# audexdev/Lossless-Audio-Codec

Measured on AMD Instinct MI355X. Metric: encode Msamples/s at 1/2/4/8 MI355X; byte-identical .lac vs CPU ref, higher is better.
Workload: dtype int64

## Files before the change

### include/lacx.h

```cpp
#ifndef LACX_H
#define LACX_H
#include <stddef.h>
#include <stdint.h>

#ifdef __cplusplus
extern "C" {
#endif

#define LACX_OK 0
#define LACX_E_INVALID 1
#define LACX_E_RUNTIME 2
#define LACX_E_DEVICE 3
#define LACX_E_MISMATCH 4

#define LACX_MAX_BLOCK 16384u
#define LACX_SLOTS_PER_BLOCK 16u

typedef struct lacx_encoder lacx_encoder;

typedef struct lacx_config {
    uint32_t sample_rate;
    uint8_t bit_depth;
    uint8_t stereo_mode;
    uint8_t zero_run_enabled;
// ... 31 lines not shown
    double h2d_ms;
    double analysis_ms;
    double ingest_ms;
    double probe_ms;
    double full_ms;
    double d2h_ms;
    double emit_ms;
    double total_ms;
    uint64_t full_slots;
    uint64_t probe_slots;
    uint32_t full_launches;
    uint32_t regrows;
    double full_exec_ms;
    uint32_t emit_direct;
    uint32_t moved_by_k_pack;
    uint32_t packer_gave_up;
    uint32_t drain_copies;
    double drain_first_ms;
    double drain_last_ms;
    double poll_gap_max_ms;
    double kernels_done_ms;
    double enqueue_ms;
    uint32_t silent_copies;
    uint32_t reserved0;
} lacx_timing;

int lacx_encoder_create(const lacx_config* cfg, lacx_encoder** out);
void lacx_encoder_destroy(lacx_encoder* enc);
const char* lacx_last_error(const lacx_encoder* enc);
void lacx_free(void* p);
void lacx_get_timing(const lacx_encoder* enc, lacx_timing* out);

uint32_t lacx_sizeof(const char* struct_name);

int lacx_encode(lacx_encoder* enc, const int32_t* left, const int32_t* right, uint64_t frames,
                uint8_t** out, uint64_t* out_size);

int lacx_encode_device(lacx_encoder* enc, const int32_t* d_left, const int32_t* d_right,
                       const int32_t* h_left, const int32_t* h_right, uint64_t frames, void* stream,
                       uint8_t** out, uint64_t* out_size);

int lacx_analyze(lacx_encoder* enc, const int32_t* left, const int32_t* right, uint64_t frames,
                 lacx_block_plan* bplans, lacx_channel_plan* plans);
int lacx_analyze_device(lacx_encoder* enc, const int32_t* d_left, const int32_t* d_right, uint64_t frames,
                        void* stream, lacx_block_plan* bplans, lacx_channel_plan* plans);

int lacx_emit_from_plans(lacx_encoder* enc, const int32_t* left, const int32_t* right, uint64_t frames,
// ... 305 lines not shown
```

### lossless-audio-codec_amd/csrc/api_core.cpp

```cpp
#include "encoder_impl.h"

namespace lacx_host {

Knobs read_knobs() {
    Knobs k;
    auto set = [](const char* name) {
        const char* v = std::getenv(name);
        return v != nullptr;
    };
    auto num = [](const char* name) -> unsigned long long {
        const char* v = std::getenv(name);
        return v ? std::strtoull(v, nullptr, 0) : 0ull;
    };
    k.stream_priority = !set("LACX_NO_STREAM_PRIORITY");
    if (const char* v = std::getenv("LACX_FUSED_EMIT")) k.fused_emit = *v != '0';
    k.direct_packer = set("LACX_DIRECT_PACKER");
    k.packer = !set("LACX_NO_PACKER");
    k.persistent = !set("LACX_NO_PERSISTENT");
    k.debug_drain = set("LACX_DEBUG_DRAIN");
    k.two_copy_streams = !set("LACX_ONE_COPY_STREAM");
    if (const char* v = std::getenv("LACX_STREAM_PRIO")) {
        int a = 0, b = 0, c = 0;
        if (std::sscanf(v, "%d,%d,%d", &a, &b, &c) == 3) {
            k.prio_main = a;
            k.prio_chunks = b;
            k.prio_pack = c;
        }
    }
    k.front_halves = !set("LACX_NO_FRONT_HALVES");
    k.tune.fold_front = !set("LACX_NO_FRONT_FOLD");
    k.lazy_repair = !set("LACX_NO_LAZY_REPAIR");
    k.silent_template = !set("LACX_NO_SILENT_TEMPLATE");
    k.pinned_cap_bytes = num("LACX_PINNED_CAP_BYTES");
    k.debug_skip = (uint32_t)num("LACX_DEBUG_SKIP");
    k.pipe_chunks = (uint32_t)num("LACX_PIPE_CHUNKS");
    if (const char* v = std::getenv("LACX_PIPE_SPLIT")) k.pipe_split = v;
    k.drain_fence = (uint32_t)num("LACX_DRAIN_FENCE");
    if (const char* v = std::getenv("LACX_FANOUT_EXCHANGE")) k.fanout_exchange = std::strcmp(v, "host") == 0 ? 1u : (std::strcmp(v, "rccl") == 0 ? 2u : 0u);
    k.tune.persistent_grid = (uint32_t)num("LACX_PERSISTENT_GRID");
    k.tune.pack_nap = (int)num("LACX_PACK_NAP");
    k.tune.pack_grid = (int)num("LACX_PACK_GRID");
    k.tune.no_pairs = set("LACX_NO_PAIRS");
    return k;
}

double ms_since(clk::time_point t0) { return std::chrono::duration<double, std::milli>(clk::now() - t0).count(); }

int fail(lacx_encoder* e, int code, const std::string& msg) {
    if (e) e->err = msg;
    return code;
}

int hip_fail(lacx_encoder* e, hipError_t err, const char* what) {
    return fail(e, LACX_E_DEVICE, std::string(what) + ": " + hipGetErrorString(err));
}

void big_copy(uint8_t* dst, const uint8_t* src, uint64_t n) {
    constexpr uint64_t kPiece = 4ull << 20;
    const unsigned hw = std::thread::hardware_concurrency();
    const uint64_t want = std::min<uint64_t>(std::min<uint64_t>(8, hw ? hw : 1), n / kPiece);
    if (want < 2) {
        std::memcpy(dst, src, n);
        return;
    }
    std::vector<std::thread> pool;
// ... 401 lines not shown
```

### lossless-audio-codec_amd/csrc/api_fanout.cpp

```cpp
#include <dlfcn.h>

#include <atomic>
#include <barrier>
#include <functional>
#include <mutex>

#include "encoder_impl.h"

namespace {
using ncclComm_t = struct ncclComm*;
using ncclResult_t = int;
constexpr int kNcclUint64 = 5;
struct Rccl {
    void* lib = nullptr;
    ncclResult_t (*CommInitAll)(ncclComm_t*, int, const int*) = nullptr;
    ncclResult_t (*CommDestroy)(ncclComm_t) = nullptr;
    ncclResult_t (*AllGather)(const void*, void*, size_t, int, ncclComm_t, hipStream_t) = nullptr;
    const char* (*GetErrorString)(ncclResult_t) = nullptr;
};
Rccl* rccl() {
    static std::mutex mu;
    static Rccl r;
    static bool tried = false;
    std::lock_guard<std::mutex> lock(mu);
// ... 202 lines not shown
    const uint32_t by_size = std::max<uint32_t>(1u, nb / std::max<uint32_t>(1u, f.min_blocks));
    return std::max<uint32_t>(1u, std::min<uint32_t>((uint32_t)f.lanes.size(), std::min(by_size, nb)));
}

void merge_timing(lacx_encoder* e, uint32_t G, clk::time_point t0) {
    lacx_timing t{};
    for (uint32_t g = 0; g < G; ++g) {
        const lacx_timing& c = e->fan->lanes[g]->enc->timing;
        t.h2d_ms = std::max(t.h2d_ms, c.h2d_ms);
        t.analysis_ms = std::max(t.analysis_ms, c.analysis_ms);
        t.ingest_ms = std::max(t.ingest_ms, c.ingest_ms);
        t.probe_ms = std::max(t.probe_ms, c.probe_ms);
        t.full_ms = std::max(t.full_ms, c.full_ms);
        t.d2h_ms = std::max(t.d2h_ms, c.d2h_ms);
        t.emit_ms = std::max(t.emit_ms, c.emit_ms);
        t.full_exec_ms = std::max(t.full_exec_ms, c.full_exec_ms);
        t.full_slots += c.full_slots;
        t.probe_slots += c.probe_slots;
        t.full_launches = std::max(t.full_launches, c.full_launches);
        t.regrows += c.regrows;
        t.emit_direct += c.emit_direct;
        t.moved_by_k_pack += c.moved_by_k_pack;
        t.silent_copies += c.silent_copies;
        t.packer_gave_up += c.packer_gave_up;
    }
    t.total_ms = ms_since(t0);
    e->timing = t;
}

}

namespace lacx_host {

bool is_fanout(const lacx_encoder* e) { return e && e->fan; }

void destroy_fanout(lacx_encoder* e) {
    if (!e->fan) return;
    Fanout* f = e->fan;
    for (size_t g = 0; g < f->lanes.size(); ++g) {
        Lane& ln = *f->lanes[g];
        ln.worker.reset();
        if (ln.comm) {
            if (Rccl* r = rccl()) (void)r->CommDestroy(ln.comm);
        }
        if (ln.d_x || ln.h_x) {
            (void)hipSetDevice(ln.device);
// ... 211 lines not shown
```

### lossless-audio-codec_amd/csrc/api_pipeline.cpp

```cpp
#include "encoder_impl.h"

namespace lacx_host {

int enqueue_chunk(lacx_encoder* e, const int32_t* d_left, const int32_t* d_right, uint64_t frames, int channels,
                  int stereo_mode, int bit_depth, const Chunk& ck, int c, hipStream_t st) {
    const uint64_t f0 = (uint64_t)ck.first * kMaxBlock;
    const uint64_t f1 = std::min<uint64_t>(frames, (uint64_t)(ck.first + ck.count) * kMaxBlock);
    const AnalyzeParams prm = make_params(e, f1 - f0, channels, stereo_mode, bit_depth);
    const DeviceWorkspace w = ws_at(e->ws, ck.first);
    LaunchSet ls = one_stream_set(prm, d_left + f0, d_right ? d_right + f0 : nullptr);
    HIP_TRY(e, launch_analysis(bind(ls), w, st, e->ev[c]), "kernel launch");
    HIP_TRY(e, hipMemcpyAsync(e->h_plans + (size_t)ck.first * kSlotsPerBlock, w.plans,
                              (size_t)ck.count * kSlotsPerBlock * sizeof(ChannelPlan), hipMemcpyDeviceToHost, st),
            "D2H plans");
    HIP_TRY(e, hipMemcpyAsync(e->h_bplans + ck.first, w.bplans, (size_t)ck.count * sizeof(BlockPlan),
                              hipMemcpyDeviceToHost, st),
            "D2H block plans");
    HIP_TRY(e, hipEventRecord(e->done[c], st), "event record");
    return LACX_OK;
}

int analyze_on_device(lacx_encoder* e, const int32_t* d_left, const int32_t* d_right, uint64_t frames,
                      int channels, int stereo_mode, int bit_depth, hipStream_t st) {
    const uint32_t nb = blocks_for(frames);
// ... 162 lines not shown
bool gather_list(lacx_encoder* e, const DeviceWorkspace& w, const GatherJob& j, GatherList& g) {
    bool ok = true;
    auto map_if = [&](bool wanted, auto* host) {
        auto* m = wanted ? mapped(host) : nullptr;
        ok = ok && (m || !wanted);
        return m;
    };
    BlockPlan* m_bplans = map_if(j.what & kGatherBplans, e->h_bplans);
    uint32_t* m_table = map_if(j.what & kGatherTable, e->h_table());
    unsigned long long* m_sizes = map_if(j.what & kGatherSizes, e->h_sizes());
    unsigned long long* m_totals = map_if(j.what & (kGatherTotal | kGatherSizes), e->h_totals);
    uint32_t* m_err = map_if(true, e->h_err);
    uint32_t* m_emitted = map_if(j.items != 0, e->h_emitted());
    unsigned long long* m_tspan = map_if(j.what & kGatherTspan, e->h_tspan);
    if (!ok) return false;
    if (m_bplans) g.add(w.bplans, m_bplans + j.first, (size_t)j.count * sizeof(BlockPlan));
    if (m_sizes) {
        g.add(e->ws.size_rec, m_sizes, (size_t)j.items * sizeof(unsigned long long));
        g.add(e->ws.size_rec, &m_totals[j.c], sizeof(unsigned long long));
    }
    if (m_table) g.add(w.table, m_table + (size_t)j.first * 2, (size_t)j.count * 2 * sizeof(uint32_t));
    if (j.what & kGatherTotal) g.add(w.block_off + j.count, &m_totals[j.c], sizeof(unsigned long long));
    g.add(w.err_flag, &m_err[j.c], sizeof(uint32_t));
    if (j.what & kGatherPacker) g.add(e->ws.err_flag + kMaxChunks, &m_err[kMaxChunks], 5 * sizeof(uint32_t));
    if (m_emitted) g.add(e->ws.packed + j.item0, m_emitted + j.item0, (size_t)j.items * sizeof(uint32_t));
    if (m_tspan) {
        g.add(w.t_first, &m_tspan[j.c], sizeof(unsigned long long));
        g.add(w.t_last, &m_tspan[kMaxChunks + j.c], sizeof(unsigned long long));
    }
    return true;
}

void fused_emit_stats(lacx_encoder* e, size_t items) {
    e->timing.emit_direct = 0;
    for (size_t i = 0; i < items; ++i) e->timing.emit_direct += e->h_emitted()[i] == 1u;
    e->timing.packer_gave_up = e->h_err[kMaxChunks + 2];
    e->timing.moved_by_k_pack = e->h_err[kMaxChunks + 3];
    e->timing.silent_copies = e->h_err[kMaxChunks + 4];
}
void add_emit_timing(lacx_encoder* e, size_t c) {
    float f = 0;
    if (hipEventElapsedTime(&f, e->ev[c][4], e->ev[c][5]) == hipSuccess) e->timing.emit_ms += f;
    (void)hipGetLastError();
    const unsigned long long a = ~e->h_tspan[c], b = e->h_tspan[kMaxChunks + c];
    if (b > a) e->timing.full_exec_ms += (double)(b - a) * 1e-5;
}

int ensure_pinned(lacx_encoder* e, uint64_t prefix, uint64_t cap, bool fresh, const char* what = nullptr) {
    if (cap > e->h_payload_cap || prefix > e->h_prefix || fresh) {
        buf_free(e->pinned);
        e->h_payload = nullptr;
        e->h_payload_cap = e->h_prefix = 0;
        if (const DevErr d = buf_grow(e->pinned, prefix + cap, 0)) return hip_fail(e, d.e, what ? what : d.what);
        e->h_payload_cap = cap;
        e->h_prefix = prefix;
    }
    e->h_payload = e->pinned.as<uint8_t>() + e->h_prefix;
    return LACX_OK;
}
int ensure_capacities(lacx_encoder* e, const Capacities& c) {
    int rc = c.dev_payload ? grow(e, e->dev_payload, c.dev_payload) : LACX_OK;
// ... 86 lines not shown
    const std::vector<ChunkPlan> chunks = e->pend.plan.chunks;
    const int dev = e->device;
    uint8_t* dst0 = const_cast<uint8_t*>(reinterpret_cast<const uint8_t*>(e->pend.d_left));
    uint8_t* dst1 = const_cast<uint8_t*>(reinterpret_cast<const uint8_t*>(e->pend.d_right));
    e->uploader->post([e, src, chunks, dev, dst0, dst1] {
        (void)hipSetDevice(dev);
        const auto tu0 = clk::now();
        bool ok = true;
        for (size_t c = 0; c < chunks.size(); ++c) {
            const uint64_t o = chunks[c].f0 * src.frame_bytes, nbytes = (chunks[c].f1 - chunks[c].f0) * src.frame_bytes;
            if (ok) ok = hipMemcpyAsync(dst0 + o, src.p0 + o, nbytes, hipMemcpyHostToDevice, e->up_stream) == hipSuccess;
            if (ok && src.p1) ok = hipMemcpyAsync(dst1 + o, src.p1 + o, nbytes, hipMemcpyHostToDevice, e->up_stream) == hipSuccess;
            if (ok) ok = hipEventRecord(e->up_ev[c], e->up_stream) == hipSuccess;
            e->up_done[c].store(ok ? 1 : -1, std::memory_order_release);
        }
        e->up_ms = ms_since(tu0);
    });
    return LACX_OK;
}

int launch_packer(lacx_encoder* e, bool persistent) {
    auto& pd = e->pend;
    const ShardPlan& p = pd.plan;
    HIP_TRY(e, hipStreamWaitEvent(e->pack_stream, e->ev[0][persistent ? 0 : 2], 0), "stream wait");
    AnalyzeParams shard_prm = make_params(e, p.in.frames, p.in.channels, p.in.stereo_mode, p.in.bit_depth, p.in.layout);
    shard_prm.stream_base = 0;
    LaunchSet shard = one_stream_set(shard_prm, nullptr, nullptr, p.fuse_items, pd.emit_cap);
    RangeProgress rp;
    if (p.drained) {
        std::memset(e->h_range(), 0, (size_t)p.ranges * sizeof(unsigned long long));
        rp.range_cnt = e->d_range_cnt;
        rp.range_end = e->d_range_end;
        HIP_TRY(e, hipHostGetDevicePointer((void**)&rp.host_end, e->h_range(), 0), "hipHostGetDevicePointer");
        rp.fuse_total = p.fuse_items;
        rp.fence_mode = e->knobs.drain_fence;
        pd.ranges = p.ranges;
    }
    HIP_TRY(e, launch_stream_out(bind(shard), e->ws, pd.emit_dst, e->ws.err_flag + kMaxChunks, e->pack_stream, rp, e->knobs.tune), "packer launch");
    HIP_TRY(e, hipEventRecord(e->pack_done, e->pack_stream), "event record");
    return LACX_OK;
}

int enqueue_analysis(lacx_encoder* e, size_t c, bool host_src) {
    auto& pd = e->pend;
    const ShardPlan& p = pd.plan;
    hipStream_t s = pd.st[p.chunks[c].stream];
    if (s != pd.st[0]) HIP_TRY(e, hipStreamWaitEvent(s, e->prologue, 0), "stream wait");
    const ChunkCtx cx = chunk_ctx(e, c);
    const FuseArgs fa = p.fused ? fuse_args(e, cx.w) : FuseArgs{};
    if (host_src) {
        const auto tw0 = clk::now();
        int st_up = 0;
        while ((st_up = e->up_done[c].load(std::memory_order_acquire)) == 0) {
            drain_pump(e);
            __builtin_ia32_pause();
            if (ms_since(tw0) > 20000.0) break;
        }
        if (st_up != 1) return fail(e, LACX_E_DEVICE, "host to device copy of the PCM failed");
        HIP_TRY(e, hipStreamWaitEvent(s, e->up_ev[c], 0), "stream wait");
    }
    LaunchSet ls = cx.set(p.chunks[c].fuse_items, pd.emit_cap);
// ... 176 lines not shown
    if (se == hipSuccess) se = se2;
    if (se != hipSuccess && status == LACX_OK) status = hip_fail(e, se, "D2H payload");
    return status;
}

int regrow(lacx_encoder* e, uint64_t* off) {
    (void)hipDeviceSynchronize();
    for (uint32_t b = 0; b < e->pend.plan.nb; ++b)
        if (e->h_bplans[b].invalid) return LACX_E_INVALID;
    const int rc = reemit_into_regrown_buffer(e, off);
    e->timing.regrows += 1;
    return rc;
}

void fill_timing(lacx_encoder* e) {
    const ShardPlan& p = e->pend.plan;
    e->timing.full_exec_ms = 0;
    for (size_t c = 0; c < p.chunks.size(); ++c) {
        add_chunk_timing(e, (int)c);
        add_emit_timing(e, c);
    }
    e->timing.full_launches = (uint32_t)p.chunks.size();
    e->timing.full_slots = (uint64_t)p.nb * (p.in.channels == 2 ? 2u : 1u);
    e->timing.emit_direct = e->timing.moved_by_k_pack = e->timing.packer_gave_up = e->timing.silent_copies = 0;
    if (p.fused) fused_emit_stats(e, (size_t)p.nb * (size_t)p.in.channels);
}

}

int encode_device_end(lacx_encoder* e, uint64_t* payload_size) {
    if (!e->pend.active) return fail(e, LACX_E_RUNTIME, "no encode in flight on this encoder");
    e->pend.active = false;
    if (e->uploader) {
        e->uploader->wait();
        if (e->up_ms > 0) e->timing.h2d_ms = e->up_ms;
        e->up_ms = 0;
    }
    const ShardPlan& p = e->pend.plan;
    if (p.drained) wait_with_drain(e);
    int status = p.lazy ? table_from_records(e) : LACX_OK;
    if (status == LACX_OK && p.lazy && e->h_err[kMaxChunks + 1] != p.nb * (uint32_t)p.in.channels) status = enqueue_repair(e);
    uint64_t off = 0;
    if (const int cs = check_chunks(e, &off)) status = cs;
    if (p.drained) status = fetch_rest(e, status, off);
    if (status == kTooSmall) status = regrow(e, &off);
    e->timing.d2h_ms = ms_since(e->pend.t0);
    if (status != LACX_OK) {
// ... 179 lines not shown
```

### lossless-audio-codec_amd/csrc/k_analyze.hip

```cpp
#include <hip/hip_runtime.h>

#include <cstdlib>
#include <mutex>

#include "emit_device.h"
#include "kernels_internal.h"

namespace lacx {

#ifdef LACX_STAMPS
__device__ unsigned long long g_stamp_acc[40];
#endif

#ifdef LACX_TEST_HOOKS
#define LACX_HOOK(prm, bits) (((prm).debug_skip & (bits)) != 0u)
#else
#define LACX_HOOK(prm, bits) false
#endif

struct PendingSlot {
    long long idx;
    uint32_t done, silent;
};

// ... 649 lines not shown
        atomicAdd(&g_stamp_acc[32], 1ull);
    }
#endif
}

#ifndef LACX_PROBE_WAVES
#define LACX_PROBE_WAVES (LACX_PROBE_HALVES ? 4 : 6)
#endif
#ifndef LACX_PROBE_WG_WAVES
#define LACX_PROBE_WG_WAVES 1
#endif
constexpr int kProbeWaves = LACX_PROBE_WG_WAVES;
constexpr int kProbeSlotsPerWave = 64 / GProbe::SW;
constexpr int kProbeSlotsPerWg = kProbeWaves * kProbeSlotsPerWave;
template <class G>
struct TailArgs {};
template <>
struct TailArgs<GProbe> {
    uint32_t* front_ctr;
    BlockPlan* bplans;
    uint32_t* need_full_out;
};
template <class G>
__global__ __launch_bounds__(G::T <= 64 ? 64 * kProbeWaves : G::T, G::T <= 64 ? LACX_PROBE_WAVES : 4) void k_analyze(BatchRef br, int probe_class, uint32_t one_block,
                                                  int which_base, const LpcSet* __restrict__ lpcs,
                                                  const uint32_t* __restrict__ need,
                                                  ChannelPlan* __restrict__ plans,
                                                  unsigned long long* __restrict__ t_first,
                                                  unsigned long long* __restrict__ t_last, FuseArgs fuse,
                                                  uint32_t* __restrict__ work_ctr, uint32_t total_wg, uint32_t pair_blocks,
                                                  TailArgs<G> tail) {
    extern __shared__ __align__(16) unsigned char smem_all[];
    __shared__ uint32_t s_next;
    __shared__ PendingSlot s_pend;
    static_assert(sizeof(Smem<G>) % 16 == 0, "slot images are 16-byte aligned");
    const int tid = G::T <= 64 ? (int)(threadIdx.x & (uint32_t)(G::SW - 1)) : (int)threadIdx.x;
    unsigned char* smem_raw = smem_all + (G::T <= 64 ? (size_t)(threadIdx.x / (uint32_t)G::SW) * sizeof(Smem<G>) : 0);
    if (t_first && tid == 0) atomicMax(t_first, ~(unsigned long long)__builtin_amdgcn_s_memrealtime());
    const bool persistent = work_ctr != nullptr;
    uint32_t rep = 0;
    uint32_t v = G::T <= 64 ? blockIdx.x * (uint32_t)kProbeWaves + (uint32_t)__builtin_amdgcn_readfirstlane((int)(threadIdx.x >> 6)) : blockIdx.x;
    if (persistent) {
        if (tid == 0) {
            s_next = atomicAdd(work_ctr, 1u);
            s_pend.idx = -1;
        }
        __syncthreads();
        v = (uint32_t)__builtin_amdgcn_readfirstlane((int)s_next);
    }
    for (;;) {
        if (persistent && v >= total_wg) break;
        uint32_t blk;
        uint32_t reps = 1u;
        int slot = -1;
        int which_in_block = -1;
        uint32_t needed_slots = 0;
        StreamDesc sd;
        if (G::SW == 32 || probe_class) {
            constexpr uint32_t kWavesPerBlock = 12u / (uint32_t)(64 / G::SW);
            blk = v / kWavesPerBlock;
            sd = stream_of_block_uniform(br, blk);
            int s = 4 + (int)(v % kWavesPerBlock) * (64 / G::SW);
            if (G::SW == 32 && upper_half()) s += 1;
            if (((uint32_t)__builtin_amdgcn_readfirstlane((int)need[blk]) >> s) & 1u) slot = s;
        } else {
            uint32_t wsel;
            if (which_base) {
                blk = one_block;
// ... 65 lines not shown
                        last = atomicAdd(&front_ctr[(size_t)blk * 2 + 1], 1u) == 11u ? 1u : 0u;
                    }
                    if (slot_first_u32<G::SW>(last)) {
                        if (tid == 0) front_ctr[(size_t)blk * 2 + 1] = 0u;
                        if (tid < 16) decide_probed_block(blk, tid, tail.bplans, tail.need_full_out, plans);
                    }
                }
            }
        }
        if (!persistent) break;
        __syncthreads();
        if (++rep < reps) continue;
        rep = 0;
        if (tid == 0) s_next = atomicAdd(work_ctr, 1u);
        __syncthreads();
        v = (uint32_t)__builtin_amdgcn_readfirstlane((int)s_next);
    }
    if (persistent) {
        asm volatile("s_waitcnt vmcnt(0)" ::: "memory");
        __syncthreads();
        publish_pending(fuse, s_pend, tid);
    }
}

size_t analyze_smem_bytes_full() { return sizeof(Smem<GFull>); }

int debug_read_stamps(unsigned long long* out32) {
#ifdef LACX_STAMPS
    if (hipMemcpyFromSymbol(out32, HIP_SYMBOL(g_stamp_acc), sizeof(unsigned long long) * 40) != hipSuccess) return 0;
    unsigned long long zero[40] = {0};
    (void)hipMemcpyToSymbol(HIP_SYMBOL(g_stamp_acc), zero, sizeof(zero));
    return 1;
#else
    (void)out32;
    return 0;
#endif
}
size_t analyze_smem_bytes_probe() { return sizeof(Smem<GProbe>) * kProbeSlotsPerWave; }

hipError_t ensure_kernel_attrs() {
    static std::mutex mu;
    static bool done[kMaxDevices] = {};
    int dev = -1;
    hipError_t e = hipGetDevice(&dev);
    if (e != hipSuccess) return e;
    if (dev < 0 || dev >= kMaxDevices) return hipErrorInvalidDevice;
// ... 143 lines not shown
```

### lossless-audio-codec_amd/csrc/k_emit.hip

```cpp
#include <hip/hip_runtime.h>

#include <cstdlib>

#include "emit_device.h"
#include "kernels_internal.h"

namespace lacx {

#ifdef LACX_STAMPS
__device__ unsigned long long g_off_stamps[8];
#define OFF_STAMP(i) do { if (threadIdx.x == 0) g_off_stamps[i] = __builtin_amdgcn_s_memrealtime(); } while (0)
#else
#define OFF_STAMP(i) do { } while (0)
#endif
__global__ __launch_bounds__(1024) void k_offsets(BatchRef br, const BlockPlan* __restrict__ bplans,
                                                   const ChannelPlan* __restrict__ plans,
                                                   unsigned long long* __restrict__ block_off,
                                                   uint32_t* __restrict__ table,
                                                   const unsigned long long* __restrict__ base_ptr,
                                                   unsigned long long* __restrict__ stream_pre) {
    __shared__ unsigned long long s_w[16];
    const int tid = threadIdx.x, lane = tid & 63, wave = tid >> 6;
    OFF_STAMP(0);
    const uint32_t nb = br.total_blocks;
// ... 149 lines not shown
            uint32_t w[5];
#pragma unroll
            for (int q = 0; q < 5; ++q) w[q] = sw32[j + q];
            uint4 o;
            o.x = __builtin_amdgcn_alignbyte(w[1], w[0], r);
            o.y = __builtin_amdgcn_alignbyte(w[2], w[1], r);
            o.z = __builtin_amdgcn_alignbyte(w[3], w[2], r);
            o.w = __builtin_amdgcn_alignbyte(w[4], w[3], r);
            vdst[v] = o;
        }
    }
    const uint32_t t0 = head + (nvec << 4);
    if (t0 + (uint32_t)tid < count) dst[t0 + tid] = src[t0 + tid];
}

#ifndef LACX_STREAM_UNROLL
#define LACX_STREAM_UNROLL 8
#endif
constexpr int kStreamGrid = 2;
constexpr int kStreamGridDevice = 3;
constexpr uint32_t kRangeItems = 256;
constexpr int kStreamThreads = 1024;
constexpr unsigned long long kStreamTimeoutTicks = 2000000ull;
__global__ __launch_bounds__(kStreamThreads) void k_stream_out(BatchRef br, uint32_t total, int nap,
                                                               const uint16_t* __restrict__ item_stream,
                                                               const unsigned long long* __restrict__ size_rec,
                                                               const unsigned long long* __restrict__ ready_rec,
                                                               const uint8_t* __restrict__ slots, unsigned long long slot_stride,
                                                               uint8_t* __restrict__ out,
                                                               uint32_t* __restrict__ packed, uint32_t* __restrict__ err_flag,
                                                               uint32_t* __restrict__ moved_total, uint32_t* __restrict__ gave_up,
                                                               RangeProgress rp) {
    const int lane = threadIdx.x & 63;
    const uint32_t unit = blockIdx.x * (uint32_t)(kStreamThreads / 64) + (threadIdx.x >> 6);
    const uint32_t units = gridDim.x * (uint32_t)(kStreamThreads / 64);
    unsigned long long running = 0;
    uint32_t summed = br.table ? 0u : br.single.prm.stream_base;
    uint32_t cur_first = summed;
    uint32_t moved = 0;
    uint32_t pend_range = 0xFFFFFFFFu, pend_count = 0;
    auto flush_progress = [&]() {
        if (pend_count == 0u) return;
        if (rp.fence_mode == 0u) __builtin_amdgcn_fence(__ATOMIC_RELEASE, "");
        else if (rp.fence_mode == 1u) __builtin_amdgcn_fence(__ATOMIC_RELEASE, "agent");
        else asm volatile("s_waitcnt vmcnt(0)" ::: "memory");
        if (lane == 0) {
            const uint32_t r = pend_range;
            const uint32_t last = (r + 1u) * kRangeItems - 1u < rp.fuse_total - 1u ? (r + 1u) * kRangeItems - 1u : rp.fuse_total - 1u;
            const uint32_t in_range = last - r * kRangeItems + 1u;
            const uint32_t before = __hip_atomic_fetch_add(&rp.range_cnt[r], pend_count, __ATOMIC_ACQ_REL, __HIP_MEMORY_SCOPE_AGENT);
            if (before + pend_count == in_range) {
                const unsigned long long end = __hip_atomic_load(&rp.range_end[r], __ATOMIC_RELAXED, __HIP_MEMORY_SCOPE_AGENT);
                __hip_atomic_store(&rp.host_end[r], end + 1ull, __ATOMIC_RELEASE, __HIP_MEMORY_SCOPE_SYSTEM);
            }
        }
        pend_count = 0;
    };
    for (uint32_t i = unit; i < total; i += units) {
        const StreamDesc sd = br.table ? br.table[item_stream[i]] : br.single;
        const uint32_t first = sd.prm.stream_base;
        if (i - first >= sd.fuse_items) continue;
        if (first != cur_first) {
            cur_first = first;
            summed = first;
            running = 0;
        }
        bool alive = true;
        unsigned long long mine = 0;
        while (alive && summed <= i) {
            const uint32_t j = summed + (uint32_t)lane;
            const unsigned long long t0 = __builtin_amdgcn_s_memrealtime();
            unsigned long long v;
            for (;;) {
                v = (j <= i) ? rec_load(&size_rec[j]) : kRecValid;
                if (__ballot((v & kRecValid) == 0ull) == 0ull) break;
                if (__builtin_amdgcn_s_memrealtime() - t0 > kStreamTimeoutTicks) {
                    alive = false;
                    break;
                }
                for (int z = 0; z < nap; ++z) __builtin_amdgcn_s_sleep(16);
            }
            if (!alive) break;
            const uint32_t cnt = (i - summed + 1u) < 64u ? (i - summed + 1u) : 64u;
            const bool last_round = summed + cnt == i + 1u;
            const bool take = (uint32_t)lane < cnt && !(last_round && (uint32_t)lane == cnt - 1u);
            running += wave_sum_u64(take ? (v & kRecBytesMask) : 0ull);
            if (last_round) mine = __shfl(v, (int)cnt - 1, 64);
            summed += cnt;
        }
        unsigned long long ready = 0;
        if (alive) {
            const unsigned long long t0 = __builtin_amdgcn_s_memrealtime();
            for (;;) {
                ready = rec_load(&ready_rec[i]);
                if (ready != 0ull) break;
                if (__builtin_amdgcn_s_memrealtime() - t0 > kStreamTimeoutTicks) {
                    alive = false;
                    break;
                }
                for (int z = 0; z < nap; ++z) __builtin_amdgcn_s_sleep(16);
            }
        }
        if (!alive) {
            if (lane == 0) atomicAdd(gave_up, 1u);
            break;
        }
        const unsigned long long off = running, rec = mine;
        running += mine & kRecBytesMask;
        if (ready == 1ull) {
            __builtin_amdgcn_fence(__ATOMIC_ACQUIRE, "agent");
            const unsigned long long bytes = rec & kRecBytesMask;
            const bool flag_byte = (rec & kRecFlag) != 0ull;
            if (off + bytes > sd.out_cap) {
                if (lane == 0) atomicOr(err_flag, 2u);
            } else {
                uint8_t* dst = out + sd.out_base + off;
                const uint32_t fb = flag_byte ? 1u : 0u;
                if (flag_byte && lane == 0) dst[0] = (rec & kRecMs) ? 1 : 0;
                copy_slot_out<64, LACX_STREAM_UNROLL>(slots + (unsigned long long)i * slot_stride, dst + fb, (uint32_t)bytes - fb, lane);
                if (lane == 0) packed[i] = 1u;
                ++moved;
            }
        } else if (lane == 0) {
            atomicOr(err_flag, 4u);
        }
        if (rp.host_end) {
            const uint32_t r = i / kRangeItems;
            if (r != pend_range) {
                flush_progress();
                pend_range = r;
            }
            const uint32_t last_of_range = (r + 1u) * kRangeItems - 1u < rp.fuse_total - 1u ? (r + 1u) * kRangeItems - 1u : rp.fuse_total - 1u;
            if (i == last_of_range && lane == 0) __hip_atomic_store(&rp.range_end[r], running, __ATOMIC_RELAXED, __HIP_MEMORY_SCOPE_AGENT);
            ++pend_count;
        }
    }
    flush_progress();
    if (lane == 0 && moved) atomicAdd(moved_total, moved);
}

constexpr int kPackGrid = 96;
__global__ __launch_bounds__(kPackThreads) void k_pack(BatchRef br, uint32_t total_items, const BlockPlan* __restrict__ bplans,
                                                       const ChannelPlan* __restrict__ plans,
                                                       const unsigned long long* __restrict__ block_off,
                                                       const uint32_t* __restrict__ table,
                                                       uint8_t* __restrict__ out,
                                                       uint32_t* __restrict__ err_flag, const uint8_t* __restrict__ slots,
                                                       unsigned long long slot_stride,
                                                       const uint32_t* __restrict__ emitted,
                                                       const uint32_t* __restrict__ packed,
                                                       const uint32_t* __restrict__ moved_total, uint32_t shard_items,
                                                       uint32_t* __restrict__ repacked) {
    if (moved_total && *moved_total == shard_items) return;
    const int tid = threadIdx.x;
    const uint32_t item0 = br.table ? br.table[0].prm.stream_base : br.single.prm.stream_base;
    for (uint32_t work = blockIdx.x; work < total_items; work += gridDim.x) {
        const size_t idx = (size_t)item0 + work;
        if (emitted[idx] != 2u || (packed && packed[idx])) continue;
        const StreamDesc sd = stream_of_item(br, (uint32_t)idx);
        const AnalyzeParams prm = sd.prm;
        const uint32_t per = prm.channels == 2 ? 2u : 1u;
        const uint32_t local = (uint32_t)idx - prm.stream_base;
// ... 67 lines not shown
        hipLaunchKernelGGL(k_pack, dim3(work < (uint32_t)kPackGrid ? work : (uint32_t)kPackGrid), dim3(kPackThreads), 0, stream, ls.br, work,
                           ws.bplans, ws.plans, ws.block_off, (const uint32_t*)ws.table, out, ws.err_flag, (const uint8_t*)ws.slots,
                           ws.slot_stride, (const uint32_t*)ws.emitted, (const uint32_t*)ws.packed, moved_total, shard_items, repacked);
    }
    const bool leftovers_only = skip_emitted && ws.slots;
    hipLaunchKernelGGL(k_emit<GFull>, dim3(leftovers_only && work > 64u ? 64u : work), dim3(GFull::T),
                       sizeof(EmitMem<GFull>), stream, ls.br, work, ws.bplans, ws.plans, ws.block_off, (const uint32_t*)ws.table,
                       out, ws.err_flag, skip_emitted ? (const uint32_t*)ws.emitted : (const uint32_t*)nullptr,
                       leftovers_only ? moved_total : (const uint32_t*)nullptr, shard_items);
    return hipGetLastError();
}

hipError_t launch_gather(const GatherList& g, hipStream_t stream) {
    if (g.n == 0) return hipSuccess;
    uint32_t most = 0;
    for (int k = 0; k < g.n; ++k) most = g.words[k] > most ? g.words[k] : most;
    const uint32_t grid = most <= 256u ? 1u : (most + 255u) / 256u > 32u ? 32u : (most + 255u) / 256u;
    hipLaunchKernelGGL(k_gather, dim3(grid), dim3(256), 0, stream, g);
    return hipGetLastError();
}

static_assert(kRangeItems == kPackerRangeItems, "host and device agree on the range size");
hipError_t launch_stream_out(const LaunchSet& ls, const DeviceWorkspace& ws, uint8_t* out, uint32_t* counters,
                             hipStream_t stream, const RangeProgress& rp, const LaunchTuning& tune) {
    if (ls.total_items == 0) return hipSuccess;
    const int nap = tune.pack_nap > 0 ? tune.pack_nap : 1;
    const int grid = tune.pack_grid > 0 ? tune.pack_grid : (rp.host_end ? kStreamGridDevice : kStreamGrid);
    hipLaunchKernelGGL(k_stream_out, dim3((uint32_t)grid), dim3(kStreamThreads), 0, stream, ls.br, ls.total_items, nap, ls.item_stream,
                       (const unsigned long long*)ws.size_rec, (const unsigned long long*)ws.ready_rec, (const uint8_t*)ws.slots,
                       ws.slot_stride, out, ws.packed, counters, counters + 1, counters + 2, rp);
    return hipGetLastError();
}

}
```

### lossless-audio-codec_amd/csrc/kernels.h

```cpp
#pragma once
#include <cstdlib>
#include <hip/hip_runtime_api.h>

#include "import_core.h"
#include "lacx_types.h"
#include "recovery_core.h"

namespace lacx {


struct DeviceWorkspace {
    ChannelPlan* plans = nullptr;
    BlockPlan* bplans = nullptr;
    uint32_t* need_probe = nullptr;
    uint32_t* need_full = nullptr;
    int64_t* acorr = nullptr;
    LpcSet* lpcs = nullptr;
    unsigned long long* sums = nullptr;
    uint32_t* badidx = nullptr;
    unsigned long long* block_off = nullptr;
    uint32_t* table = nullptr;
    uint32_t* err_flag = nullptr;
    unsigned long long* t_first = nullptr;
    unsigned long long* t_last = nullptr;
    uint32_t* front_ctr = nullptr;
    uint32_t* work_ctr = nullptr;
    uint8_t* slots = nullptr;
    unsigned long long slot_stride = 0;
    uint32_t* emitted = nullptr;
    uint32_t* packed = nullptr;
    unsigned long long* size_rec = nullptr;
    unsigned long long* ready_rec = nullptr;
    unsigned long long* stream_pre = nullptr;
};

inline bool analysis_is_persistent(const DeviceWorkspace& ws) { return ws.work_ctr != nullptr; }

struct LaunchTuning {
    uint32_t persistent_grid = 0;
    int pack_nap = 0;
    int pack_grid = 0;
    bool fold_front = true;
    bool no_pairs = false;
    hipStream_t aux_stream = nullptr;
    hipEvent_t aux_ev[2] = {nullptr, nullptr};
};

struct RangeProgress {
    uint32_t* range_cnt = nullptr;
    unsigned long long* range_end = nullptr;
    unsigned long long* host_end = nullptr;
    uint32_t fuse_total = 0;
    uint32_t fence_mode = 0;
};
constexpr uint32_t kPackerRangeItems = 256;

struct LaunchSet {
    BatchRef br;
    const StreamDesc* streams = nullptr;
    uint32_t nstreams = 0;
    uint32_t total_items = 0;
    const uint16_t* item_stream = nullptr;
};
inline LaunchSet single_set(const StreamDesc& sd) {
// ... 35 lines not shown
    uint32_t words[kMax];
    int n = 0;
    void add(const void* s, void* d, size_t bytes) {
        src[n] = s;
        dst[n] = d;
        words[n] = (uint32_t)(bytes / 4);
        ++n;
    }
};
hipError_t launch_gather(const GatherList& g, hipStream_t stream);

hipError_t launch_analysis(const LaunchSet& ls, const DeviceWorkspace& ws, hipStream_t stream, hipEvent_t* ev,
                           const FuseArgs* fuse = nullptr, hipEvent_t wait_before_full = nullptr,
                           const LaunchTuning& tune = LaunchTuning{});

hipError_t launch_emit(const LaunchSet& ls, const DeviceWorkspace& ws, uint8_t* out,
                       const unsigned long long* base_ptr, hipEvent_t wait_before_offsets,
                       hipEvent_t offsets_done, hipStream_t stream, bool skip_emitted = true,
                       const uint32_t* moved_total = nullptr, uint32_t shard_items = 0,
                       hipEvent_t wait_before_pack = nullptr, uint32_t* repacked = nullptr, bool lazy_repair = false);

hipError_t launch_stream_out(const LaunchSet& ls, const DeviceWorkspace& ws, uint8_t* out, uint32_t* counters,
                             hipStream_t stream, const RangeProgress& rp = RangeProgress{},
                             const LaunchTuning& tune = LaunchTuning{});

hipError_t launch_decode(const DecodeArgs& args, hipStream_t stream);

hipError_t launch_digest(const DecodeArgs& args, hipStream_t stream);
hipError_t launch_digest_pcm(const DigestPcmArgs& args, hipStream_t stream);

hipError_t launch_digest_blocks(const DecodeArgs& args, hipStream_t stream);
hipError_t launch_digest_pcm_blocks(const BlockPcmArgs& args, hipStream_t stream);

hipError_t launch_recovery(const RecoveryArgs& args, hipStream_t stream);

hipError_t launch_wide_block(const int32_t* d_x, uint32_t n, int zero_run, int partitioning, int32_t* d_res,
                             ChannelPlan* d_plan, hipStream_t stream);

hipError_t launch_import(const ImportJob& job, ImportBad* bad, hipStream_t stream);

size_t analyze_smem_bytes_full();
int debug_read_stamps(unsigned long long* out32);
int debug_read_offset_stamps(unsigned long long* out8);
size_t analyze_smem_bytes_probe();

}
```

### lossless-audio-codec_amd/lacx.py

```python
from __future__ import annotations

import ctypes as C
import os
import subprocess

import numpy as np

HERE = os.path.dirname(os.path.abspath(__file__))
LIB_PATH = os.path.join(HERE, "liblacx.so")
HOOKS_LIB_PATH = os.path.join(HERE, "liblacx_hooks.so")
DEVICE_ALL = -2
MAX_FANOUT = 16

OK, E_INVALID, E_RUNTIME, E_DEVICE, E_MISMATCH = 0, 1, 2, 3, 4
MAX_BLOCK = 16384
SLOTS = 16
CH_L, CH_R, CH_M, CH_S = 0, 1, 2, 3


class Config(C.Structure):
    _fields_ = [
        ("sample_rate", C.c_uint32),
        ("bit_depth", C.c_uint8),
        ("stereo_mode", C.c_uint8),
# ... 35 lines not shown
        ("h2d_ms", C.c_double),
        ("analysis_ms", C.c_double),
        ("ingest_ms", C.c_double),
        ("probe_ms", C.c_double),
        ("full_ms", C.c_double),
        ("d2h_ms", C.c_double),
        ("emit_ms", C.c_double),
        ("total_ms", C.c_double),
        ("full_slots", C.c_uint64),
        ("probe_slots", C.c_uint64),
        ("full_launches", C.c_uint32),
        ("regrows", C.c_uint32),
        ("full_exec_ms", C.c_double),
        ("emit_direct", C.c_uint32),
        ("moved_by_k_pack", C.c_uint32),
        ("packer_gave_up", C.c_uint32),
        ("drain_copies", C.c_uint32),
        ("drain_first_ms", C.c_double),
        ("drain_last_ms", C.c_double),
        ("poll_gap_max_ms", C.c_double),
        ("kernels_done_ms", C.c_double),
        ("enqueue_ms", C.c_double),
        ("silent_copies", C.c_uint32),
        ("reserved0", C.c_uint32),
    ]


EXPORTS = (
    "lacx_encoder_create", "lacx_encoder_destroy", "lacx_last_error", "lacx_free", "lacx_get_timing",
    "lacx_encode", "lacx_encode_device", "lacx_analyze", "lacx_analyze_device", "lacx_emit_from_plans",
    "lacx_encode_shard", "lacx_encode_shard_device", "lacx_encode_shard_device_view", "lacx_encode_shard_pcm_device_view", "lacx_assemble", "lacx_block_encode",
    "lacx_block_plan_only", "lacx_debug_lpc", "lacx_debug_stamps", "lacx_device_count", "lacx_wav_parse",
    "lacx_encode_wav", "lacx_encode_shard_pcm_device_begin", "lacx_encode_shard_end", "lacx_debug_emit_workers", "lacx_encode_wav_view",
    "lacx_stream_parse", "lacx_decode", "lacx_decode_last_error", "lacx_encode_batch_device",
    "lacx_encoder_create_multi", "lacx_encoder_lanes", "lacx_fanout_range", "lacx_encode_fanout_resident",
    "lacx_get_fanout_stats", "lacx_get_lane_timing", "lacx_fanout_exchange_note",
    "lacx_decoder_create", "lacx_decoder_destroy", "lacx_decoder_decode", "lacx_sizeof",
    "lacx_decoder_decode_wav", "lacx_decoder_decode_wav_view",
    "lacx_decoder_decode_wav_batch", "lacx_decoder_decode_wav_batch_view", "lacx_decoder_decode_batch_device",
    "lacx_decoder_item_error", "lacx_decoder_decode_window_batch_device", "lacx_decoder_decode_window",
    "lacx_decoder_verify_batch_device", "lacx_decoder_verify_wav",
    "lacx_decoder_digest_batch_device", "lacx_decoder_digest_pcm_batch_device", "lacx_crc32_combine",
    "lacx_stream_scan", "lacx_decoder_salvage_wav_batch_view", "lacx_decoder_salvage_wav",
    "lacx_decoder_salvage_batch_device", "lacx_decoder_item_faults", "lacx_block_fault_text",
    "lacx_decoder_digest_blocks_batch_device", "lacx_decoder_item_block_digests", "lacx_decoder_digest_pcm_blocks_batch_device",
    "lacx_manifest_build", "lacx_manifest_parse", "lacx_decoder_check_batch_device",
    "lacx_decoder_salvage_wav_batch_view_checked", "lacx_decoder_salvage_batch_device_checked",
# ... 1387 lines not shown
```

Baseline: 24990.

## Add slim single-wave persistent packer and cap analyze VGPRs for co-residency

Adds a slim stream-out packer kernel that runs one 64-thread wave per workgroup with a 16-VGPR cap, wave-uniform scalarized loads, and a smaller unroll. It is launched by default with 48 waves for drained persistent shards, and can wait on the later event. Separately, the full analyze kernel gets a VGPR cap so more workgroups can be resident alongside the packer. A counter of analysis workgroups is added to the timing struct. The aim is to stop the packer from stealing compute from analysis while it overlaps, at the risk of register spills and a slower copy phase.

```diff
diff --git a/include/lacx.h b/include/lacx.h
--- a/include/lacx.h
+++ b/include/lacx.h
@@ -77,7 +77,7 @@
     double kernels_done_ms;
     double enqueue_ms;
     uint32_t silent_copies;
-    uint32_t reserved0;
+    uint32_t analysis_wgs;
 } lacx_timing;
 
 int lacx_encoder_create(const lacx_config* cfg, lacx_encoder** out);
diff --git a/lossless-audio-codec_amd/csrc/api_core.cpp b/lossless-audio-codec_amd/csrc/api_core.cpp
--- a/lossless-audio-codec_amd/csrc/api_core.cpp
+++ b/lossless-audio-codec_amd/csrc/api_core.cpp
@@ -41,6 +41,8 @@
     k.tune.pack_nap = (int)num("LACX_PACK_NAP");
     k.tune.pack_grid = (int)num("LACX_PACK_GRID");
     k.tune.no_pairs = set("LACX_NO_PAIRS");
+    if (set("LACX_PACK_WAVES")) k.tune.pack_waves = (int)std::min<unsigned long long>(num("LACX_PACK_WAVES"), 1024ull);
+    if (const char* v = std::getenv("LACX_PACK_LATE")) k.tune.pack_late = *v != '0';
     return k;
 }
 
diff --git a/lossless-audio-codec_amd/csrc/api_fanout.cpp b/lossless-audio-codec_amd/csrc/api_fanout.cpp
--- a/lossless-audio-codec_amd/csrc/api_fanout.cpp
+++ b/lossless-audio-codec_amd/csrc/api_fanout.cpp
@@ -248,6 +248,7 @@
         t.emit_direct += c.emit_direct;
         t.moved_by_k_pack += c.moved_by_k_pack;
         t.silent_copies += c.silent_copies;
+        t.analysis_wgs += c.analysis_wgs;
         t.packer_gave_up += c.packer_gave_up;
     }
     t.total_ms = ms_since(t0);
diff --git a/lossless-audio-codec_amd/csrc/api_pipeline.cpp b/lossless-audio-codec_amd/csrc/api_pipeline.cpp
--- a/lossless-audio-codec_amd/csrc/api_pipeline.cpp
+++ b/lossless-audio-codec_amd/csrc/api_pipeline.cpp
@@ -208,7 +208,7 @@
     if (m_table) g.add(w.table, m_table + (size_t)j.first * 2, (size_t)j.count * 2 * sizeof(uint32_t));
     if (j.what & kGatherTotal) g.add(w.block_off + j.count, &m_totals[j.c], sizeof(unsigned long long));
     g.add(w.err_flag, &m_err[j.c], sizeof(uint32_t));
-    if (j.what & kGatherPacker) g.add(e->ws.err_flag + kMaxChunks, &m_err[kMaxChunks], 5 * sizeof(uint32_t));
+    if (j.what & kGatherPacker) g.add(e->ws.err_flag + kMaxChunks, &m_err[kMaxChunks], 6 * sizeof(uint32_t));
     if (m_emitted) g.add(e->ws.packed + j.item0, m_emitted + j.item0, (size_t)j.items * sizeof(uint32_t));
     if (m_tspan) {
         g.add(w.t_first, &m_tspan[j.c], sizeof(unsigned long long));
@@ -223,6 +223,7 @@
     e->timing.packer_gave_up = e->h_err[kMaxChunks + 2];
     e->timing.moved_by_k_pack = e->h_err[kMaxChunks + 3];
     e->timing.silent_copies = e->h_err[kMaxChunks + 4];
+    e->timing.analysis_wgs = e->h_err[kMaxChunks + 5];
 }
 void add_emit_timing(lacx_encoder* e, size_t c) {
     float f = 0;
@@ -355,7 +356,8 @@
 int launch_packer(lacx_encoder* e, bool persistent) {
     auto& pd = e->pend;
     const ShardPlan& p = pd.plan;
-    HIP_TRY(e, hipStreamWaitEvent(e->pack_stream, e->ev[0][persistent ? 0 : 2], 0), "stream wait");
+    const bool slim = persistent && p.drained && e->knobs.tune.pack_waves > 0;
+    HIP_TRY(e, hipStreamWaitEvent(e->pack_stream, e->ev[0][persistent && !(slim && e->knobs.tune.pack_late) ? 0 : 2], 0), "stream wait");
     AnalyzeParams shard_prm = make_params(e, p.in.frames, p.in.channels, p.in.stereo_mode, p.in.bit_depth, p.in.layout);
     shard_prm.stream_base = 0;
     LaunchSet shard = one_stream_set(shard_prm, nullptr, nullptr, p.fuse_items, pd.emit_cap);
@@ -369,7 +371,7 @@
         rp.fence_mode = e->knobs.drain_fence;
         pd.ranges = p.ranges;
     }
-    HIP_TRY(e, launch_stream_out(bind(shard), e->ws, pd.emit_dst, e->ws.err_flag + kMaxChunks, e->pack_stream, rp, e->knobs.tune), "packer launch");
+    HIP_TRY(e, launch_stream_out(bind(shard), e->ws, pd.emit_dst, e->ws.err_flag + kMaxChunks, e->pack_stream, rp, e->knobs.tune, slim), "packer launch");
     HIP_TRY(e, hipEventRecord(e->pack_done, e->pack_stream), "event record");
     return LACX_OK;
 }
@@ -592,7 +594,7 @@
     }
     e->timing.full_launches = (uint32_t)p.chunks.size();
     e->timing.full_slots = (uint64_t)p.nb * (p.in.channels == 2 ? 2u : 1u);
-    e->timing.emit_direct = e->timing.moved_by_k_pack = e->timing.packer_gave_up = e->timing.silent_copies = 0;
+    e->timing.emit_direct = e->timing.moved_by_k_pack = e->timing.packer_gave_up = e->timing.silent_copies = e->timing.analysis_wgs = 0;
     if (p.fused) fused_emit_stats(e, (size_t)p.nb * (size_t)p.in.channels);
 }
 
diff --git a/lossless-audio-codec_amd/csrc/k_analyze.hip b/lossless-audio-codec_amd/csrc/k_analyze.hip
--- a/lossless-audio-codec_amd/csrc/k_analyze.hip
+++ b/lossless-audio-codec_amd/csrc/k_analyze.hip
@@ -695,7 +695,7 @@
     uint32_t* need_full_out;
 };
 template <class G>
-__global__ __launch_bounds__(G::T <= 64 ? 64 * kProbeWaves : G::T, G::T <= 64 ? LACX_PROBE_WAVES : 4) void k_analyze(BatchRef br, int probe_class, uint32_t one_block,
+__device__ __forceinline__ void analyze_kernel_body(BatchRef br, int probe_class, uint32_t one_block,
                                                   int which_base, const LpcSet* __restrict__ lpcs,
                                                   const uint32_t* __restrict__ need,
                                                   ChannelPlan* __restrict__ plans,
@@ -717,6 +717,7 @@
         if (tid == 0) {
             s_next = atomicAdd(work_ctr, 1u);
             s_pend.idx = -1;
+            if (s_next < total_wg && fuse.silent_copies) atomicAdd(fuse.silent_copies + 1, 1u);
         }
         __syncthreads();
         v = (uint32_t)__builtin_amdgcn_readfirstlane((int)s_next);
@@ -828,6 +829,28 @@
         publish_pending(fuse, s_pend, tid);
     }
 }
+
+#define LACX_ANALYZE_ARGS                                                                                              \
+    BatchRef br, int probe_class, uint32_t one_block, int which_base, const LpcSet *__restrict__ lpcs,                 \
+        const uint32_t *__restrict__ need, ChannelPlan *__restrict__ plans, unsigned long long *__restrict__ t_first,  \
+        unsigned long long *__restrict__ t_last, FuseArgs fuse, uint32_t *__restrict__ work_ctr, uint32_t total_wg,    \
+        uint32_t pair_blocks
+#define LACX_ANALYZE_PASS br, probe_class, one_block, which_base, lpcs, need, plans, t_first, t_last, fuse, work_ctr, total_wg, pair_blocks, tail
+template <class G>
+__global__ __launch_bounds__(G::T <= 64 ? 64 * kProbeWaves : G::T, G::T <= 64 ? LACX_PROBE_WAVES : 4) void k_analyze(LACX_ANALYZE_ARGS, TailArgs<G> tail) {
+    analyze_kernel_body<G>(LACX_ANALYZE_PASS);
+}
+#ifndef LACX_ANALYZE_VGPR_CAP
+#define LACX_ANALYZE_VGPR_CAP 120
+#endif
+#if LACX_ANALYZE_VGPR_CAP
+template <>
+__global__ __launch_bounds__(GFull::T, 4) __attribute__((amdgpu_num_vgpr(LACX_ANALYZE_VGPR_CAP / 2))) void k_analyze<GFull>(LACX_ANALYZE_ARGS, TailArgs<GFull> tail) {
+    analyze_kernel_body<GFull>(LACX_ANALYZE_PASS);
+}
+#endif
+#undef LACX_ANALYZE_ARGS
+#undef LACX_ANALYZE_PASS
 
 size_t analyze_smem_bytes_full() { return sizeof(Smem<GFull>); }
 
diff --git a/lossless-audio-codec_amd/csrc/k_emit.hip b/lossless-audio-codec_amd/csrc/k_emit.hip
--- a/lossless-audio-codec_amd/csrc/k_emit.hip
+++ b/lossless-audio-codec_amd/csrc/k_emit.hip
@@ -195,20 +195,23 @@
 constexpr uint32_t kRangeItems = 256;
 constexpr int kStreamThreads = 1024;
 constexpr unsigned long long kStreamTimeoutTicks = 2000000ull;
-__global__ __launch_bounds__(kStreamThreads) void k_stream_out(BatchRef br, uint32_t total, int nap,
-                                                               const uint16_t* __restrict__ item_stream,
-                                                               const unsigned long long* __restrict__ size_rec,
-                                                               const unsigned long long* __restrict__ ready_rec,
-                                                               const uint8_t* __restrict__ slots, unsigned long long slot_stride,
-                                                               uint8_t* __restrict__ out,
-                                                               uint32_t* __restrict__ packed, uint32_t* __restrict__ err_flag,
-                                                               uint32_t* __restrict__ moved_total, uint32_t* __restrict__ gave_up,
-                                                               RangeProgress rp) {
+#define LACX_STREAM_OUT_ARGS                                                                                           \
+    BatchRef br, uint32_t total, int nap, const uint16_t *__restrict__ item_stream,                                    \
+        const unsigned long long *__restrict__ size_rec, const unsigned long long *__restrict__ ready_rec,             \
+        const uint8_t *__restrict__ slots, unsigned long long slot_stride, uint8_t *__restrict__ out,                  \
+        uint32_t *__restrict__ packed, uint32_t *__restrict__ err_flag, uint32_t *__restrict__ moved_total,            \
+        uint32_t *__restrict__ gave_up, RangeProgress rp
+#define LACX_STREAM_OUT_PASS br, total, nap, item_stream, size_rec, ready_rec, slots, slot_stride, out, packed, err_flag, moved_total, gave_up, rp
+__device__ __forceinline__ unsigned long long wave_uniform_u64(unsigned long long v) {
+    const uint32_t lo = (uint32_t)__builtin_amdgcn_readfirstlane((int)(uint32_t)v);
+    const uint32_t hi = (uint32_t)__builtin_amdgcn_readfirstlane((int)(uint32_t)(v >> 32));
+    return ((unsigned long long)hi << 32) | lo;
+}
+template <int UNROLL, bool SCALAR>
+__device__ __forceinline__ void stream_out_wave(LACX_STREAM_OUT_ARGS, const uint32_t unit, const uint32_t units) {
     const int lane = threadIdx.x & 63;
-    const uint32_t unit = blockIdx.x * (uint32_t)(kStreamThreads / 64) + (threadIdx.x >> 6);
-    const uint32_t units = gridDim.x * (uint32_t)(kStreamThreads / 64);
     unsigned long long running = 0;
-    uint32_t summed = br.table ? 0u : br.single.prm.stream_base;
+    uint32_t summed = (!SCALAR && br.table) ? 0u : br.single.prm.stream_base;
     uint32_t cur_first = summed;
     uint32_t moved = 0;
     uint32_t pend_range = 0xFFFFFFFFu, pend_count = 0;
@@ -230,7 +233,7 @@
         pend_count = 0;
     };
     for (uint32_t i = unit; i < total; i += units) {
-        const StreamDesc sd = br.table ? br.table[item_stream[i]] : br.single;
+        const StreamDesc sd = (!SCALAR && br.table) ? br.table[item_stream[i]] : br.single;
         const uint32_t first = sd.prm.stream_base;
         if (i - first >= sd.fuse_items) continue;
         if (first != cur_first) {
@@ -259,6 +262,7 @@
             const bool take = (uint32_t)lane < cnt && !(last_round && (uint32_t)lane == cnt - 1u);
             running += wave_sum_u64(take ? (v & kRecBytesMask) : 0ull);
             if (last_round) mine = __shfl(v, (int)cnt - 1, 64);
+            if (SCALAR) mine = wave_uniform_u64(mine);
             summed += cnt;
         }
         unsigned long long ready = 0;
@@ -266,6 +270,7 @@
             const unsigned long long t0 = __builtin_amdgcn_s_memrealtime();
             for (;;) {
                 ready = rec_load(&ready_rec[i]);
+                if (SCALAR) ready = wave_uniform_u64(ready);
                 if (ready != 0ull) break;
                 if (__builtin_amdgcn_s_memrealtime() - t0 > kStreamTimeoutTicks) {
                     alive = false;
@@ -290,7 +295,7 @@
                 uint8_t* dst = out + sd.out_base + off;
                 const uint32_t fb = flag_byte ? 1u : 0u;
                 if (flag_byte && lane == 0) dst[0] = (rec & kRecMs) ? 1 : 0;
-                copy_slot_out<64, LACX_STREAM_UNROLL>(slots + (unsigned long long)i * slot_stride, dst + fb, (uint32_t)bytes - fb, lane);
+                copy_slot_out<64, UNROLL>(slots + (unsigned long long)i * slot_stride, dst + fb, (uint32_t)bytes - fb, lane);
                 if (lane == 0) packed[i] = 1u;
                 ++moved;
             }
@@ -311,6 +316,18 @@
     flush_progress();
     if (lane == 0 && moved) atomicAdd(moved_total, moved);
 }
+__global__ __launch_bounds__(kStreamThreads) void k_stream_out(LACX_STREAM_OUT_ARGS) {
+    stream_out_wave<LACX_STREAM_UNROLL, false>(LACX_STREAM_OUT_PASS, blockIdx.x * (uint32_t)(kStreamThreads / 64) + (threadIdx.x >> 6),
+                                        gridDim.x * (uint32_t)(kStreamThreads / 64));
+}
+#ifndef LACX_STREAM_UNROLL_SLIM
+#define LACX_STREAM_UNROLL_SLIM 2
+#endif
+__global__ __launch_bounds__(64) __attribute__((amdgpu_num_vgpr(16))) void k_stream_out_slim(LACX_STREAM_OUT_ARGS) {
+    stream_out_wave<LACX_STREAM_UNROLL_SLIM, true>(LACX_STREAM_OUT_PASS, blockIdx.x, gridDim.x);
+}
+#undef LACX_STREAM_OUT_ARGS
+#undef LACX_STREAM_OUT_PASS
 
 constexpr int kPackGrid = 96;
 __global__ __launch_bounds__(kPackThreads) void k_pack(BatchRef br, uint32_t total_items, const BlockPlan* __restrict__ bplans,
@@ -424,9 +441,16 @@
 
 static_assert(kRangeItems == kPackerRangeItems, "host and device agree on the range size");
 hipError_t launch_stream_out(const LaunchSet& ls, const DeviceWorkspace& ws, uint8_t* out, uint32_t* counters,
-                             hipStream_t stream, const RangeProgress& rp, const LaunchTuning& tune) {
+                             hipStream_t stream, const RangeProgress& rp, const LaunchTuning& tune, bool slim) {
     if (ls.total_items == 0) return hipSuccess;
     const int nap = tune.pack_nap > 0 ? tune.pack_nap : 1;
+    if (slim) {
+        if (ls.br.table != nullptr || tune.pack_waves <= 0) return hipErrorInvalidValue;
+        hipLaunchKernelGGL(k_stream_out_slim, dim3((uint32_t)tune.pack_waves), dim3(64), 0, stream, ls.br, ls.total_items, nap, ls.item_stream,
+                           (const unsigned long long*)ws.size_rec, (const unsigned long long*)ws.ready_rec, (const uint8_t*)ws.slots,
+                           ws.slot_stride, out, ws.packed, counters, counters + 1, counters + 2, rp);
+        return hipGetLastError();
+    }
     const int grid = tune.pack_grid > 0 ? tune.pack_grid : (rp.host_end ? kStreamGridDevice : kStreamGrid);
     hipLaunchKernelGGL(k_stream_out, dim3((uint32_t)grid), dim3(kStreamThreads), 0, stream, ls.br, ls.total_items, nap, ls.item_stream,
                        (const unsigned long long*)ws.size_rec, (const unsigned long long*)ws.ready_rec, (const uint8_t*)ws.slots,
diff --git a/lossless-audio-codec_amd/csrc/kernels.h b/lossless-audio-codec_amd/csrc/kernels.h
--- a/lossless-audio-codec_amd/csrc/kernels.h
+++ b/lossless-audio-codec_amd/csrc/kernels.h
@@ -40,6 +40,8 @@
     uint32_t persistent_grid = 0;
     int pack_nap = 0;
     int pack_grid = 0;
+    int pack_waves = 48;
+    bool pack_late = true;
     bool fold_front = true;
     bool no_pairs = false;
     hipStream_t aux_stream = nullptr;
@@ -121,7 +123,7 @@
 
 hipError_t launch_stream_out(const LaunchSet& ls, const DeviceWorkspace& ws, uint8_t* out, uint32_t* counters,
                              hipStream_t stream, const RangeProgress& rp = RangeProgress{},
-                             const LaunchTuning& tune = LaunchTuning{});
+                             const LaunchTuning& tune = LaunchTuning{}, bool slim = false);
 
 hipError_t launch_decode(const DecodeArgs& args, hipStream_t stream);
 
diff --git a/lossless-audio-codec_amd/lacx.py b/lossless-audio-codec_amd/lacx.py
--- a/lossless-audio-codec_amd/lacx.py
+++ b/lossless-audio-codec_amd/lacx.py
@@ -81,7 +81,7 @@
         ("kernels_done_ms", C.c_double),
         ("enqueue_ms", C.c_double),
         ("silent_copies", C.c_uint32),
-        ("reserved0", C.c_uint32),
+        ("analysis_wgs", C.c_uint32),
     ]
 
 
```

New measurement: 25070, median of 6. Within noise of the previous version (+0.3%).
